# czbiohub-sf/yogo

Hardware: AMD Instinct MI355X
Metric: training images/sec (772x1032 gray) (higher is better)
Workload: dtype bf16; 1 GPU; BASELINE configs[2]: full train step (fwd+loss+bwd+clamp+AdamW), base_model, 772x1032x1 uint8, 7 classes; per_gpu_batch=128, global_batch=128, parallelism=dp1

## Files before the change

yogo_amd/csrc/conv_bf16_direct.hip:

```cpp
#include "common.h"
#ifndef YOGO_ST_AUX
#define YOGO_ST_AUX 2
#endif
#include <mutex>

#ifndef DD_ABL
#define DD_ABL 0
#endif
typedef unsigned int u32x4 __attribute__((ext_vector_type(4)));
typedef float f32x16 __attribute__((ext_vector_type(16)));
typedef __bf16 bf16x8 __attribute__((ext_vector_type(8)));

struct ConvDirectS2dParams {
  const u32x4* in;
  const u32x4* wp;
  u32x4* out;
  const unsigned char* signs;
  const float* chan_scale;
  int B, Kb, M, Mb, Mpad, IH, IW, OH, OW;
  int npass;
  int tiles_per_img, ntiles;
  unsigned m_iw, m_tpi;
};

namespace {
__device__ __forceinline__ int dd_udivm1(int n, int d, unsigned m) { return d == 1 ? n : (int)__umulhi((unsigned)n, m); }
}

template <int NK, int NMB, bool SIGNS>
__global__ __launch_bounds__(256 * NMB) __attribute__((amdgpu_waves_per_eu(NMB == 1 ? 4 : 2, NMB == 1 ? 4 : 2))) void conv_bf16_s2d_direct_kernel(
    const ConvDirectS2dParams p) {
  extern __shared__ __attribute__((aligned(16))) u32x4 lds_w[];
  constexpr int OOB = (int)0x80000000u;
  constexpr int KB = 2 * NK, MP = 32 * NMB, NT = 256 * NMB, NWV = 4 * NMB;
  const int tid = threadIdx.x, lane = tid & 63, l31 = lane & 31, half = lane >> 5;
  const int wave = __builtin_amdgcn_readfirstlane(tid >> 6);
  const int bid = blockIdx.x;
  const int xcd = bid & 7;
  const int pass = (bid >> 3) % p.npass;
  const int slot = bid / (8 * p.npass);
  const int nslot = gridDim.x / (8 * p.npass);
  const int t8 = (p.ntiles + 7) >> 3;
  const int t_end = min(p.ntiles, (xcd + 1) * t8);
  for (int i = tid; i < 9 * KB * MP; i += NT) {
    const int m = i % MP, r = i / MP;
    lds_w[i] = p.wp[(size_t)r * p.Mpad + pass * MP + m];
  }
  float* my_scale = reinterpret_cast<float*>(lds_w + 9 * KB * MP) + wave * MP;
  __syncthreads();
  const int IH = p.IH, IW = p.IW, OH = p.OH, OW = p.OW;
  const int kcb = IH * IW * 16, plane = OH * OW, plane16 = plane * 16, nq = IH * IW;
  const int sq = p.Mpad >> 4;
  const int ch0 = pass * MP;
  struct Geo {
    int b, pix;
    int vsh[4];
    bool qv, vx, vy;
  };
  auto geo_of = [&](int tile) __attribute__((always_inline)) {
    Geo g;
    g.b = dd_udivm1(tile, p.tiles_per_img, p.m_tpi);
    const int t = tile - g.b * p.tiles_per_img;
    const int q = t * 32 + l31;
    g.qv = q < nq;
    const int qc = g.qv ? q : nq - 1;
    const int a = dd_udivm1(qc, IW, p.m_iw), c = qc - a * IW;
    const bool cx = c + 1 < IW, cy = a + 1 < IH;
    g.vx = 2 * c + 1 < OW; g.vy = 2 * a + 1 < OH;
    const int v00 = (a * IW + c) * 16 + half * kcb;
    g.vsh[0] = v00; g.vsh[1] = cx ? v00 + 16 : OOB; g.vsh[2] = cy ? v00 + IW * 16 : OOB; g.vsh[3] = (cx && cy) ? v00 + IW * 16 + 16 : OOB;
    g.pix = 2 * a * OW + 2 * c;
    return g;
  };
  u32x4 Bq[2][4];
  auto load_step = [&](const Geo& g, int kc, u32x4 (&dst)[4]) __attribute__((always_inline)) {
    const auto rs_in = __builtin_amdgcn_make_buffer_rsrc((void*)(p.in + (size_t)g.b * KB * IH * IW), (short)0, KB * kcb, 0x00020000);
#pragma unroll
    for (int s = 0; s < 4; ++s) dst[s] = __builtin_bit_cast(u32x4, __builtin_amdgcn_raw_buffer_load_b128(rs_in, (DD_ABL & 4) ? OOB : g.vsh[s], (2 * kc) * kcb, 0));
  };
  static_assert(NK % 2 == 0, "the first operand set of the NEXT tile is requested while the last step still reads the second");
  const int tstep = nslot * NWV;
  int tile = xcd * t8 + slot * NWV + wave;
  Geo G = geo_of(min(tile, p.ntiles - 1));
  if (tile < t_end) load_step(G, 0, Bq[0]);
  for (; tile < t_end; tile += tstep) {
    const int b = G.b, pix = G.pix;
    const bool qv = G.qv, vx = G.vx, vy = G.vy;
    const auto rs_o = __builtin_amdgcn_make_buffer_rsrc((void*)(p.out + (size_t)b * p.Mb * plane), (short)0, p.Mb * plane16, 0x00020000);
    float my_s = 0.f;
    if (lane < MP) my_s = ch0 + lane < p.M ? (p.chan_scale != nullptr ? p.chan_scale[(size_t)b * p.M + ch0 + lane] : 1.f) : 0.f;
    unsigned sg[2][2] = {{0u, 0u}, {0u, 0u}};
    if constexpr (SIGNS) {
      const auto rs_s = __builtin_amdgcn_make_buffer_rsrc((void*)(p.signs + (size_t)b * plane * 2 * sq), (short)0, plane * 2 * sq, 0x00020000);
#pragma unroll
      for (int py = 0; py < 2; ++py)
#pragma unroll
        for (int px = 0; px < 2; ++px) {
          const bool ok = qv && (px == 0 || vx) && (py == 0 || vy);
          const int vs = ok ? (half * plane + pix + py * OW + px) * sq + pass * 2 * NMB : OOB;
          if constexpr (NMB == 2) sg[py][px] = (unsigned)__builtin_amdgcn_raw_buffer_load_b32(rs_s, vs, 0, 0);
          else sg[py][px] = (unsigned)__builtin_amdgcn_raw_buffer_load_b16(rs_s, vs, 0, 0);
        }
    }
    f32x16 acc[NMB][2][2];
#pragma unroll
    for (int mb = 0; mb < NMB; ++mb)
#pragma unroll
      for (int py = 0; py < 2; ++py)
#pragma unroll
        for (int px = 0; px < 2; ++px)
#pragma unroll
          for (int r = 0; r < 16; ++r) acc[mb][py][px][r] = 0.f;
#pragma unroll
    for (int kc = 0; kc < NK; ++kc) {
      if (kc + 1 < NK) load_step(G, kc + 1, Bq[(kc + 1) & 1]);
      const u32x4(&Bc)[4] = Bq[kc & 1];
      const u32x4* wk = lds_w + (2 * kc + half) * MP + l31;
#define DD_MF(PY, PX, S, SH)                                                                                                                     \
  _Pragma("unroll") for (int mb = 0; mb < NMB; ++mb) if (!(DD_ABL & 2)) acc[mb][PY][PX] = __builtin_amdgcn_mfma_f32_32x32x16_bf16(               \
      __builtin_bit_cast(bf16x8, (DD_ABL & 8) ? Bc[(SH) ^ 1] : wk[(S) * KB * MP + 32 * mb]), __builtin_bit_cast(bf16x8, Bc[SH]), acc[mb][PY][PX], 0, 0, 0); \
  else acc[mb][PY][PX][0] += __builtin_bit_cast(float, Bc[SH].x);
      __builtin_amdgcn_sched_barrier(0);
      DD_MF(0, 0, 0, 0) DD_MF(0, 1, 1, 0) DD_MF(1, 0, 3, 0)
      __builtin_amdgcn_sched_barrier(0);
      DD_MF(1, 1, 5, 0) DD_MF(0, 1, 2, 1) DD_MF(1, 1, 6, 1)
      __builtin_amdgcn_sched_barrier(0);
      DD_MF(1, 0, 4, 2) DD_MF(1, 1, 7, 2) DD_MF(1, 1, 8, 3)
      __builtin_amdgcn_sched_barrier(0);
#undef DD_MF
    }
    __builtin_amdgcn_sched_barrier(0);
    if (tile + tstep < t_end) {
      G = geo_of(tile + tstep);
      load_step(G, 0, Bq[0]);
    }
    __builtin_amdgcn_sched_barrier(0);
    if (lane < MP) my_scale[lane] = my_s;
#pragma unroll
    for (int mb = 0; mb < NMB; ++mb)
#pragma unroll
    for (int gp = 0; gp < 2; ++gp) {
      const int cb = pass * 4 * NMB + 4 * mb + 2 * gp;
      const int cl = 32 * mb + 16 * gp + 4 * half;
      const float4 sA = *reinterpret_cast<const float4*>(my_scale + cl), sB = *reinterpret_cast<const float4*>(my_scale + cl + 8);
      const float sa[8] = {sA.x, sA.y, sA.z, sA.w, sB.x, sB.y, sB.z, sB.w};
      float sl[8];
#pragma unroll
      for (int i = 0; i < 8; ++i) sl[i] = LEAKY_SLOPE * sa[i];
#pragma unroll
      for (int py = 0; py < 2; ++py) {
        u32x4 un[2];
#pragma unroll
        for (int px = 0; px < 2; ++px) {
          float v[8];
          if constexpr (SIGNS) {
            const unsigned m = sg[py][px] >> (8 * (2 * mb + gp));
#pragma unroll
            for (int i = 0; i < 8; ++i) {
              const int tt = (int)(m << (31 - i)) >> 31;
              unsigned f;
              asm("v_bfi_b32 %0, %1, %2, %3" : "=v"(f) : "v"(tt), "v"(sa[i]), "v"(sl[i]));
              v[i] = acc[mb][py][px][8 * gp + i] * __builtin_bit_cast(float, f);
            }
          } else {
#pragma unroll
            for (int i = 0; i < 8; ++i) v[i] = fmaf(acc[mb][py][px][8 * gp + i], sa[i], 0.f * sa[i]);
          }
          bf16x8 o;
#pragma unroll
          for (int i = 0; i < 8; ++i) o[i] = (__bf16)v[i];
          const u32x4 w = __builtin_bit_cast(u32x4, o);
          const auto r0 = __builtin_amdgcn_permlane32_swap(w.x, w.z, false, false);
          const auto r1 = __builtin_amdgcn_permlane32_swap(w.y, w.w, false, false);
          un[px] = u32x4{r0[0], r1[0], r0[1], r1[1]};
        }
        u32x4 se[2];
        {
          const auto x0 = __builtin_amdgcn_permlane32_swap(un[0].x, un[1].x, false, false);
          const auto x1 = __builtin_amdgcn_permlane32_swap(un[0].y, un[1].y, false, false);
          const auto x2 = __builtin_amdgcn_permlane32_swap(un[0].z, un[1].z, false, false);
          const auto x3 = __builtin_amdgcn_permlane32_swap(un[0].w, un[1].w, false, false);
          se[0] = u32x4{x0[0], x1[0], x2[0], x3[0]};
          se[1] = u32x4{x0[1], x1[1], x2[1], x3[1]};
        }
        const bool okp = qv && (half == 0 || vx) && (py == 0 || vy);
#pragma unroll
        for (int e = 0; e < 2; ++e)
          __builtin_amdgcn_raw_buffer_store_b128(se[e], rs_o, (okp && cb + e < p.Mb && !(DD_ABL & 1)) ? (pix + py * OW + half) * 16 + (cb + e) * plane16 : OOB, 0, YOGO_ST_AUX);
      }
    }
  }
}

bool conv_bf16_s2d_direct_eligible(int K, int M, int OH, int OW, int B) {
  if (M < 1 || !((M <= 32 && (K == 32 || K == 64)) || (M > 64 && M <= 128 && K == 128))) return false;
  if (OH < 2 || OW < 2 || B <= 0) return false;
  const long long IH = (OH + 1) / 2, IW = (OW + 1) / 2, Mb = ((M + 15) / 16) * 2;
  if ((long long)(K / 8) * IH * IW * 16 >= (1ll << 31) || Mb * OH * OW * 16 >= (1ll << 31) || (long long)B * ((IH * IW + 31) / 32) >= (1ll << 31)) return false;
  const long long tpi = (IH * IW + 31) / 32;
  if (!magic_div_exact(B * tpi - 1, (int)tpi) || !magic_div_exact(tpi * 32, (int)IW)) return false;
  return true;
}

int launch_conv_bf16_s2d_direct(const void* in, const void* packed, void* out, const void* signs, const float* chan_scale, int B, int K, int M, int IH, int IW,
                                int OH, int OW, hipStream_t stream) {
  static std::mutex mu;
  static int n_cu_of[64] = {0};
  static bool attr_set[64] = {false};
  int dev = 0;
  if (hipGetDevice(&dev) != hipSuccess || dev < 0 || dev >= 64) {
    yogo_set_error("conv_bf16_s2d_direct: hipGetDevice failed");
    return YOGO_ERR_HIP;
  }
  const int nmb = M <= 32 ? 1 : 2;
  const int lds = 9 * (K / 8) * 32 * nmb * 16 + 4 * nmb * 32 * nmb * 4;
  int n_cu;
  {
    std::lock_guard<std::mutex> lk(mu);
    if (n_cu_of[dev] == 0) {
      hipDeviceProp_t prop;
      n_cu_of[dev] = (hipGetDeviceProperties(&prop, dev) == hipSuccess && prop.multiProcessorCount > 0) ? prop.multiProcessorCount : 256;
    }
    n_cu = n_cu_of[dev];
    if (nmb == 2 && !attr_set[dev]) {
      hipError_t e = hipFuncSetAttribute(reinterpret_cast<const void*>(&conv_bf16_s2d_direct_kernel<8, 2, true>), hipFuncAttributeMaxDynamicSharedMemorySize, lds);
      if (e == hipSuccess) e = hipFuncSetAttribute(reinterpret_cast<const void*>(&conv_bf16_s2d_direct_kernel<8, 2, false>), hipFuncAttributeMaxDynamicSharedMemorySize, lds);
      if (e != hipSuccess) {
        yogo_set_error("conv_bf16_s2d_direct: hipFuncSetAttribute: %s", hipGetErrorString(e));
        return YOGO_ERR_HIP;
      }
      attr_set[dev] = true;
    }
  }
  ConvDirectS2dParams p{};
  p.in = reinterpret_cast<const u32x4*>(in); p.wp = reinterpret_cast<const u32x4*>(packed); p.out = reinterpret_cast<u32x4*>(out);
  p.signs = reinterpret_cast<const unsigned char*>(signs); p.chan_scale = chan_scale;
  p.B = B; p.Kb = K / 8; p.M = M; p.Mb = ((M + 15) / 16) * 2; p.Mpad = nmb == 1 ? 32 : 128; p.IH = IH; p.IW = IW; p.OH = OH; p.OW = OW;
  p.npass = p.Mpad / (32 * nmb);
  p.tiles_per_img = cdiv(IH * IW, 32);
  p.ntiles = B * p.tiles_per_img;
  auto magic = [](int d) -> unsigned { return d <= 1 ? 0xFFFFFFFFu : (unsigned)(((1ull << 32) + (unsigned)d - 1ull) / (unsigned)d); };
  p.m_iw = magic(IW); p.m_tpi = magic(p.tiles_per_img);
  if (p.ntiles <= 0) return YOGO_OK;
  const int t8 = cdiv(p.ntiles, 8);
  const int grid = nmb == 1 ? 8 * max(1, min(cdiv(t8, 4), 4 * n_cu / 8)) : 16 * max(1, min(cdiv(t8, 8), n_cu / 16));
  const bool sg = signs != nullptr;
#define DD_LAUNCH(NK, NMB, S) hipLaunchKernelGGL((conv_bf16_s2d_direct_kernel<NK, NMB, S>), dim3(grid), dim3(256 * NMB), lds, stream, p)
  if (K == 128) { if (sg) DD_LAUNCH(8, 2, true); else DD_LAUNCH(8, 2, false); }
  else if (K == 64) { if (sg) DD_LAUNCH(4, 1, true); else DD_LAUNCH(4, 1, false); }
  else { if (sg) DD_LAUNCH(2, 1, true); else DD_LAUNCH(2, 1, false); }
#undef DD_LAUNCH
  if (yogo_launch_log_enabled())
    yogo_launch_log("conv_bf16_s2d_direct_kernel<%d, %d, %s> | K=%d M=%d dy=%dx%d dx=%dx%d tiles=%d grid=%d lds=%d signs=%d scale=%d", K / 16, nmb, sg ? "true" : "false",
                    K, M, IH, IW, OH, OW, p.ntiles, grid, lds, sg, chan_scale != nullptr);
  YOGO_CHECK_LAUNCH("conv_bf16_s2d_direct");
  return YOGO_OK;
}
```

yogo_amd/csrc/conv_first_fused_bwd.hip:

```cpp
#include "common.h"
#include <mutex>
#include <type_traits>
#include <utility>

typedef unsigned int u32x4 __attribute__((ext_vector_type(4)));
typedef int i32x4 __attribute__((ext_vector_type(4)));
typedef float f32x4 __attribute__((ext_vector_type(4)));
typedef float f32x2 __attribute__((ext_vector_type(2)));
typedef __bf16 bf16x8 __attribute__((ext_vector_type(8)));

struct DgFirstParams {
  const u32x4* g;
  const u32x4* wp;
  const unsigned char* img;
  const unsigned short* signs;
  float* part;
  const u32x4* x;
  float* slab;
  float* bias_part;
  int B, H, W, Mpad, act, ncol;
  int tiles_per_row, tile_rows, seg, segs_per_img, nsegs;
  unsigned m_tpr, m_spi;
};

namespace {
constexpr int DF_NJ = 9, DF_PER = 2 * DF_NJ + 2, DF_COUT = 16;
__device__ __forceinline__ int df_udivm1(int n, int d, unsigned m) { return d == 1 ? n : (int)__umulhi((unsigned)n, m); }
__device__ __forceinline__ unsigned df_u(unsigned v) { return (unsigned)__builtin_amdgcn_readfirstlane((int)v); }
__device__ __forceinline__ i32x4 df_rsrc(const void* ptr, unsigned bytes) {
  const unsigned long long a = reinterpret_cast<unsigned long long>(ptr);
  return i32x4{(int)df_u((unsigned)a), (int)df_u((unsigned)(a >> 32) & 0xFFFFu), (int)df_u(bytes), 0x00020000};
}
__device__ __forceinline__ void df_dma16(i32x4 rs, unsigned lds_addr, int voff) {
  unsigned keep;
  lds_addr = df_u(lds_addr);
  asm volatile("s_mov_b32 %0, m0\n\ts_mov_b32 m0, %2\n\ts_nop 4\n\tbuffer_load_dwordx4 %1, %3, 0 offen lds\n\ts_mov_b32 m0, %0"
               : "=&s"(keep) : "v"(voff), "s"(lds_addr), "s"(rs) : "memory");
}
__device__ __forceinline__ void df_dma4(i32x4 rs, unsigned lds_addr, int voff) {
  unsigned keep;
  lds_addr = df_u(lds_addr);
  asm volatile("s_mov_b32 %0, m0\n\ts_mov_b32 m0, %2\n\ts_nop 4\n\tbuffer_load_dword %1, %3, 0 offen lds\n\ts_mov_b32 m0, %0"
               : "=&s"(keep) : "v"(voff), "s"(lds_addr), "s"(rs) : "memory");
}
__device__ __forceinline__ void df_wait_dma() { asm volatile("s_waitcnt vmcnt(0)" ::: "memory"); }
__device__ __forceinline__ bf16x8 df_tr8(const unsigned char* a, int second) {
  typedef __bf16 bf16x4 __attribute__((ext_vector_type(4)));
  typedef bf16x4 __attribute__((address_space(3))) * lds_v4;
  const bf16x4 lo = __builtin_amdgcn_ds_read_tr16_b64_v4bf16((lds_v4)(a));
  const bf16x4 hi = __builtin_amdgcn_ds_read_tr16_b64_v4bf16((lds_v4)(a + second));
  return __builtin_shufflevector(lo, hi, 0, 1, 2, 3, 4, 5, 6, 7);
}
}

#ifndef DF_WAVES_PER_EU
#define DF_WAVES_PER_EU 2
#endif
#ifndef DF_NPF
#define DF_NPF 6
#endif
#ifndef DF_NPF_WG
#define DF_NPF_WG 3
#endif
namespace {
template <class F, int... I>
__device__ __forceinline__ void df_static_for(F&& f, std::integer_sequence<int, I...>) {
  (f(std::integral_constant<int, I>{}), ...);
}
}
template <int R, int NWV, bool WG>
__global__ __launch_bounds__(64 * NWV) __attribute__((amdgpu_waves_per_eu(DF_WAVES_PER_EU))) void conv_bf16_dgrad_first_bwd_kernel(const DgFirstParams p) {
  extern __shared__ __attribute__((aligned(16))) u32x4 lds_u[];
  constexpr int OOB = (int)0x80000000u;
  constexpr int KB = 4, NR = R + 2, ROWU = 34, TU = KB * NR * ROWU, NDMA = (TU + 63) / 64;
  constexpr int IR = 2 * R + 1, IROWB = 72, IDW = IROWB / 4, IU = IR * IDW, NIDMA = (IU + 63) / 64;
  constexpr int SU = R * 16, NSDMA = (SU + 63) / 64;
  static_assert(!WG || (R % 2) == 0, "a piece of the staged x tile is two whole rows");
  constexpr int NXDMA = WG ? R : 0;
  constexpr int WAVE_BYTES = NDMA * 1024 + NIDMA * 256 + NSDMA * 256 + NXDMA * 1024;
  constexpr int CONST_BYTES = ((IR * IROWB + 15) / 16) * 16;
  const int tid = threadIdx.x, lane = tid & 63, c16 = lane & 15, g4 = lane >> 4;
  const int wave = __builtin_amdgcn_readfirstlane(tid >> 6);
  const int H = p.H, W = p.W, IH0 = 2 * H, IW0 = 2 * W;
  const int kcb = H * W * 16;
  const bool leaky = p.act == ACT_LEAKY;
  const unsigned my_addr = (unsigned)(wave * WAVE_BYTES), my_img_addr = my_addr + NDMA * 1024, my_sg_addr = my_img_addr + NIDMA * 256;
  [[maybe_unused]] const unsigned my_x_addr = my_sg_addr + NSDMA * 256;
  const unsigned ones_addr = (unsigned)(NWV * WAVE_BYTES), zeros_addr = ones_addr + CONST_BYTES;
  const u32x4* my_tile = lds_u + wave * (WAVE_BYTES / 16);
  const unsigned char* lds8 = reinterpret_cast<const unsigned char*>(lds_u);
  {
    unsigned* cw = reinterpret_cast<unsigned*>(lds_u) + ones_addr / 4;
    for (int e = tid; e < CONST_BYTES / 4; e += 64 * NWV) {
      cw[e] = 0x01010101u;
      cw[e + CONST_BYTES / 4] = 0u;
    }
  }
  __syncthreads();

  bf16x8 wv[9];
#pragma unroll
  for (int tp = 0; tp < 9; ++tp) wv[tp] = __builtin_bit_cast(bf16x8, p.wp[(tp * KB + g4) * p.Mpad + c16]);

  int rel[NDMA];
  unsigned rc[NDMA];
#pragma unroll
  for (int i = 0; i < NDMA; ++i) {
    const int u = i * 64 + lane;
    const int kb = u / (NR * ROWU), rem = u - kb * (NR * ROWU);
    const int r = rem / ROWU, cc = rem - r * ROWU;
    rel[i] = u < TU ? kb * kcb + (r * W + cc) * 16 : OOB;
    rc[i] = u < TU ? (unsigned)(r << 16 | cc) : 0xFFFFFFFFu;
  }
  unsigned irc[NIDMA];
#pragma unroll
  for (int i = 0; i < NIDMA; ++i) {
    const int e = i * 64 + lane;
    const int r = e / IDW, d = e - r * IDW;
    irc[i] = e < IU ? (unsigned)(r << 16 | d) : 0xFFFFFFFFu;
  }
  const int xj = c16 < 9 ? c16 : 0, kh = xj / 3, kw = xj - 3 * kh;
  const unsigned x_addr = c16 < 9 ? my_img_addr + (unsigned)(kh * IROWB + ((3 + 8 * g4 + kw) & ~3)) : (c16 == 9 ? ones_addr : zeros_addr) + (unsigned)(8 * g4);
  const unsigned x_sh = c16 < 9 ? (unsigned)((3 + kw) & 3) : 0u;
  const unsigned sg_addr = my_sg_addr + (unsigned)(8 * g4);
  const unsigned sg_pos = (unsigned)(c16 < 4 ? c16 : c16 < 8 ? c16 + 4 : c16 < 12 ? c16 - 4 : c16);

  f32x4 d2p = {0.f, 0.f, 0.f, 0.f}, d2n = {0.f, 0.f, 0.f, 0.f};
  f32x4 wacc[WG ? 2 : 1][WG ? 9 : 1], bacc[WG ? 2 : 1];
#pragma unroll
  for (int c = 0; c < (WG ? 2 : 1); ++c) {
    bacc[c] = f32x4{0.f, 0.f, 0.f, 0.f};
#pragma unroll
    for (int t = 0; t < (WG ? 9 : 1); ++t) wacc[c][t] = f32x4{0.f, 0.f, 0.f, 0.f};
  }
  [[maybe_unused]] const unsigned tr_g = my_addr + (unsigned)((((c16 & 3) >> 1) * NR * ROWU + 8 * g4 + (c16 >> 2)) * 16 + (c16 & 1) * 8);
  [[maybe_unused]] const unsigned tr_x = my_x_addr + (unsigned)((((c16 & 3) >> 1) * R * 32 + 8 * g4 + (c16 >> 2)) * 16 + (c16 & 1) * 8);
  const u32x4 ones_op = {0x3F803F80u, 0x3F803F80u, 0x3F803F80u, 0x3F803F80u};

  const int xcd = blockIdx.x & 7, slot = blockIdx.x >> 3, nslot = gridDim.x >> 3;
  const int s8 = (p.nsegs + 7) >> 3, s_end = min(p.nsegs, (xcd + 1) * s8);
  for (int sgm = xcd * s8 + slot * NWV + wave; sgm < s_end; sgm += nslot * NWV) {
    const int b = df_udivm1(sgm, p.segs_per_img, p.m_spi);
    const int t = sgm - b * p.segs_per_img;
    const int sy = df_udivm1(t, p.tiles_per_row, p.m_tpr), ox0 = (t - sy * p.tiles_per_row) * 32;
    const int ty_end = min(p.tile_rows, (sy + 1) * p.seg);
   for (int ty = sy * p.seg; ty < ty_end; ++ty) {
    const int oy0 = ty * R;
    {
      const i32x4 rs_g = df_rsrc(p.g + (size_t)b * KB * H * W, (unsigned)(KB * kcb));
      const int iy0 = oy0 - 1, ix0 = ox0 - 1;
      const int base = (iy0 * W + ix0) * 16;
      if (iy0 >= 0 && iy0 + NR <= H && ix0 >= 0 && ix0 + ROWU <= W) {
#pragma unroll
        for (int i = 0; i < NDMA; ++i) df_dma16(rs_g, my_addr + (unsigned)i * 1024u, (i + 1) * 64 <= TU ? rel[i] + base : (rel[i] == OOB ? OOB : rel[i] + base));
      } else {
#pragma unroll
        for (int i = 0; i < NDMA; ++i) {
          const int r = (int)(rc[i] >> 16), c = (int)(rc[i] & 0xFFFFu);
          const bool ok = ((unsigned)(iy0 + r) < (unsigned)H) && ((unsigned)(ix0 + c) < (unsigned)W);
          df_dma16(rs_g, my_addr + (unsigned)i * 1024u, ok ? rel[i] + base : OOB);
        }
      }
      const i32x4 rs_i = df_rsrc(p.img + (size_t)b * IH0 * IW0, (unsigned)(IH0 * IW0));
      const int jy0 = 2 * oy0 - 1, jx0 = 2 * ox0 - 4;
#pragma unroll
      for (int i = 0; i < NIDMA; ++i) {
        const int r = (int)(irc[i] >> 16), d = (int)(irc[i] & 0xFFFFu);
        const int iy = jy0 + r, ix = jx0 + 4 * d;
        const bool ok = ((unsigned)iy < (unsigned)IH0) && ((unsigned)ix < (unsigned)IW0);
        df_dma4(rs_i, my_img_addr + (unsigned)i * 256u, ok ? iy * IW0 + ix : OOB);
      }
      if (leaky) {
        const i32x4 rs_s = df_rsrc(p.signs + (size_t)b * H * W, (unsigned)(H * W * 2));
#pragma unroll
        for (int i = 0; i < NSDMA; ++i) {
          const int e = i * 64 + lane, r = e >> 4, d = e & 15;
          const bool ok = e < SU && oy0 + r < H && ox0 + 2 * d < W;
          df_dma4(rs_s, my_sg_addr + (unsigned)i * 256u, ok ? ((oy0 + r) * W + ox0 + 2 * d) * 2 : OOB);
        }
      }
      if constexpr (WG) {
        const i32x4 rs_x = df_rsrc(p.x + (size_t)b * 2 * H * W, (unsigned)(2 * kcb));
        const int hi = lane >> 5, col = lane & 31;
        const int xo = ((oy0 + hi) * W + ox0 + col) * 16;
        const bool cok = ox0 + col < W;
#pragma unroll
        for (int i = 0; i < NXDMA; ++i) {
          constexpr int dummy = 0; (void)dummy;
          const int kb = (2 * i) / R, row0 = (2 * i) % R;
          df_dma16(rs_x, my_x_addr + (unsigned)i * 1024u, (cok && oy0 + row0 + hi < H) ? xo + kb * kcb + row0 * W * 16 : OOB);
        }
      }
    }
    const bool right = ox0 + 32 > W;
    df_wait_dma();
    const u32x4* bt = my_tile + g4 * NR * ROWU + c16;
#pragma unroll
    for (int rr = 0; rr < R; ++rr) {
      if (oy0 + rr >= H) break;
      constexpr int NST = WG ? 36 : 18, NPF = WG ? DF_NPF_WG : DF_NPF;
      f32x4 acc[2];
      bf16x8 ring[NPF];
      [[maybe_unused]] bf16x8 xt;
      auto load = [&](auto s_tag) {
        constexpr int S = decltype(s_tag)::value;
        if constexpr (S < 18) {
          constexpr int pb = S / 9, tp = S % 9, ky = tp / 3, kx = tp % 3;
          ring[S % NPF] = __builtin_bit_cast(bf16x8, bt[(rr + ky) * ROWU + 16 * pb + kx]);
        } else {
          constexpr int cbk = (S - 18) / 9, tp = (S - 18) % 9, ky = tp / 3, kx = tp % 3;
          ring[S % NPF] = df_tr8(lds8 + tr_g + ((cbk * 2 * NR + rr + 2 - ky) * ROWU + 2 - kx) * 16, 64);
        }
      };
      auto use = [&](auto s_tag) {
        constexpr int S = decltype(s_tag)::value;
        if constexpr (S < 18) {
          constexpr int pb = S / 9, tp = S % 9;
          acc[pb] = __builtin_amdgcn_mfma_f32_16x16x32_bf16(ring[S % NPF], wv[tp], tp == 0 ? f32x4{0.f, 0.f, 0.f, 0.f} : acc[pb], 0, 0, 0);
        } else if constexpr (WG) {
          constexpr int cbk = (S - 18) / 9, tp = (S - 18) % 9;
          wacc[cbk][tp] = __builtin_amdgcn_mfma_f32_16x16x32_bf16(ring[S % NPF], xt, wacc[cbk][tp], 0, 0, 0);
          if constexpr (tp == 4) bacc[cbk] = __builtin_amdgcn_mfma_f32_16x16x32_bf16(ring[S % NPF], __builtin_bit_cast(bf16x8, ones_op), bacc[cbk], 0, 0, 0);
        }
      };
      unsigned xr[2][3];
      unsigned sw[2][2] = {{0xFFFFFFFFu, 0xFFFFFFFFu}, {0xFFFFFFFFu, 0xFFFFFFFFu}};
      u32x4 xop, gpos, gneg;
      auto p3 = [&](auto k_tag) {
        constexpr int K = decltype(k_tag)::value;
        typedef __bf16 bf16x2 __attribute__((ext_vector_type(2)));
        if constexpr (K == 0) {
#pragma unroll
          for (int pb = 0; pb < 2; ++pb) {
            const unsigned char* xa = lds8 + x_addr + rr * (2 * IROWB) + 32 * pb;
            xr[pb][0] = *reinterpret_cast<const unsigned*>(xa);
            xr[pb][1] = *reinterpret_cast<const unsigned*>(xa + 4);
            xr[pb][2] = *reinterpret_cast<const unsigned*>(xa + 8);
            if (leaky) {
              const unsigned long long s2 = *reinterpret_cast<const unsigned long long*>(lds8 + sg_addr + rr * 64 + 32 * pb);
              sw[pb][0] = (unsigned)s2;
              sw[pb][1] = (unsigned)(s2 >> 32);
            }
          }
        } else if constexpr (K == 1 || K == 2) {
          constexpr int pb = K - 1;
          const unsigned lo4 = __builtin_amdgcn_alignbyte(xr[pb][1], xr[pb][0], x_sh), hi4 = __builtin_amdgcn_alignbyte(xr[pb][2], xr[pb][1], x_sh);
          const unsigned xs = __builtin_amdgcn_perm(hi4, lo4, 0x06040200u);
          const bf16x2 q0 = {(__bf16)(float)(xs & 0xFFu), (__bf16)(float)((xs >> 8) & 0xFFu)};
          const bf16x2 q1 = {(__bf16)(float)((xs >> 16) & 0xFFu), (__bf16)(float)(xs >> 24)};
          xop[2 * pb] = __builtin_bit_cast(unsigned, q0);
          xop[2 * pb + 1] = __builtin_bit_cast(unsigned, q1);
        } else if constexpr (K == 3 || K == 4) {
          constexpr int pb = K - 3;
#pragma unroll
          for (int q = 0; q < 2; ++q) {
            const bf16x2 dq = {(__bf16)acc[pb][2 * q], (__bf16)acc[pb][2 * q + 1]};
            unsigned dw = __builtin_bit_cast(unsigned, dq);
            if (right && ox0 + 16 * pb + 4 * g4 + 2 * q >= W) dw = 0u;
            const unsigned m = leaky ? __umul24((sw[pb][q] >> sg_pos) & 0x00010001u, 0xFFFFu) : 0xFFFFFFFFu;
            const unsigned pos = dw & m;
            gpos[2 * pb + q] = pos;
            gneg[2 * pb + q] = dw ^ pos;
          }
        } else if constexpr (K == 5) {
          d2p = __builtin_amdgcn_mfma_f32_16x16x32_bf16(__builtin_bit_cast(bf16x8, xop), __builtin_bit_cast(bf16x8, gpos), d2p, 0, 0, 0);
        } else {
          d2n = __builtin_amdgcn_mfma_f32_16x16x32_bf16(__builtin_bit_cast(bf16x8, xop), __builtin_bit_cast(bf16x8, gneg), d2n, 0, 0, 0);
        }
      };
      df_static_for([&](auto s_tag) { load(s_tag); }, std::make_integer_sequence<int, NPF>{});
      __builtin_amdgcn_sched_barrier(0);
      df_static_for(
          [&](auto s_tag) {
            constexpr int S = decltype(s_tag)::value;
            use(s_tag);
            if constexpr (S + NPF < NST) load(std::integral_constant<int, S + NPF>{});
            if constexpr (WG) {
              if constexpr (S == 10) xt = df_tr8(lds8 + tr_x + rr * 512, 64);
              if constexpr (S == 18) p3(std::integral_constant<int, 0>{});
              if constexpr (S == 23) p3(std::integral_constant<int, 1>{});
              if constexpr (S == 25) p3(std::integral_constant<int, 2>{});
              if constexpr (S == 27) p3(std::integral_constant<int, 3>{});
              if constexpr (S == 29) p3(std::integral_constant<int, 4>{});
              if constexpr (S == 31) p3(std::integral_constant<int, 5>{});
              if constexpr (S == 32) p3(std::integral_constant<int, 6>{});
            } else {
              if constexpr (S == 12) p3(std::integral_constant<int, 0>{});
              if constexpr (S == 15) p3(std::integral_constant<int, 1>{});
              if constexpr (S == 16) p3(std::integral_constant<int, 2>{});
            }
            __builtin_amdgcn_sched_barrier(0);
          },
          std::make_integer_sequence<int, NST>{});
      if constexpr (!WG) {
        p3(std::integral_constant<int, 3>{});
        p3(std::integral_constant<int, 4>{});
        p3(std::integral_constant<int, 5>{});
        p3(std::integral_constant<int, 6>{});
      }
    }
   }
  }
  float* prow = p.part + (size_t)(blockIdx.x * NWV + wave) * p.ncol;
#pragma unroll
  for (int i = 0; i < 4; ++i) {
    const int j = 4 * g4 + i;
    const float v = d2p[i] + LEAKY_SLOPE * d2n[i];
    if (j < DF_NJ) prow[c16 * DF_PER + j] = v;
    else if (j == DF_NJ) prow[c16 * DF_PER + 2 * DF_NJ] = v;
  }
  if (g4 == 0) prow[c16 * DF_PER + 2 * DF_NJ + 1] = 0.f;
  for (int e = lane; e < DF_COUT * DF_NJ; e += 64) prow[(e / DF_NJ) * DF_PER + DF_NJ + e % DF_NJ] = 0.f;
  for (int e = lane; e < DF_NJ + DF_NJ * DF_NJ; e += 64) prow[DF_COUT * DF_PER + e] = 0.f;
  if constexpr (WG) {
    constexpr int NE = 9 * 32 * 16, STRIDE = NE + 32;
    static_assert(NWV * STRIDE * 4 <= NWV * WAVE_BYTES + 2 * CONST_BYTES, "the reduction uses the kernel's LDS allocation");
    __syncthreads();
    float* red = reinterpret_cast<float*>(lds_u) + wave * STRIDE;
#pragma unroll
    for (int cbk = 0; cbk < 2; ++cbk)
#pragma unroll
      for (int i = 0; i < 4; ++i) {
        const int co = 16 * cbk + 4 * g4 + i;
#pragma unroll
        for (int tp = 0; tp < 9; ++tp) red[(tp * 32 + co) * 16 + c16] = wacc[cbk][tp][i];
        if (c16 == 0) red[NE + co] = bacc[cbk][i];
      }
    __syncthreads();
    const float* r0 = reinterpret_cast<const float*>(lds_u);
    float* sl = p.slab + (size_t)blockIdx.x * NE;
    float* bp = p.bias_part + (size_t)blockIdx.x * 32;
    for (int e = tid; e < STRIDE; e += 64 * NWV) {
      float v = r0[e];
#pragma unroll
      for (int w = 1; w < NWV; ++w) v += r0[w * STRIDE + e];
      if (e < NE) sl[e] = v;
      else bp[e - NE] = v;
    }
  }
}

#ifndef DF_TILE_ROWS
#define DF_TILE_ROWS 6
#endif
#ifndef DF_TILE_ROWS_WG
#define DF_TILE_ROWS_WG 4
#endif
#ifndef DF_WAVES
#define DF_WAVES 4
#endif
namespace {
constexpr int DF_NWV = DF_WAVES;
constexpr int df_rows(bool wg) { return wg ? DF_TILE_ROWS_WG : DF_TILE_ROWS; }
constexpr int df_lds_bytes(int R, int NWV, bool wg) {
  return NWV * (((4 * (R + 2) * 34 + 63) / 64) * 1024 + (((2 * R + 1) * 18 + 63) / 64) * 256 + ((R * 16 + 63) / 64) * 256 + (wg ? R * 1024 : 0)) +
         2 * ((((2 * R + 1) * 72 + 15) / 16) * 16);
}
int df_n_cu() {
  static std::mutex mu;
  static int n_cu_of[64] = {0};
  int dev = 0;
  if (hipGetDevice(&dev) != hipSuccess || dev < 0 || dev >= 64) return -1;
  std::lock_guard<std::mutex> lk(mu);
  if (n_cu_of[dev] == 0) {
    hipDeviceProp_t prop;
    n_cu_of[dev] = (hipGetDeviceProperties(&prop, dev) == hipSuccess && prop.multiProcessorCount > 0) ? prop.multiProcessorCount : 256;
  }
  return n_cu_of[dev];
}
struct DfPlan { int grid, seg; };
DfPlan df_plan(int B, int H, int W, int n_cu, bool wg) {
  const int R = df_rows(wg);
  const int nty = cdiv(H, R), ntx = cdiv(W, 32);
  const int lds = df_lds_bytes(R, DF_NWV, wg);
  const int per_cu = max(1, min(16 / DF_NWV, (160 * 1024) / lds));
#ifdef DF_SEG
  const int seg_lo = DF_SEG, seg_hi = DF_SEG;
#else
  const int seg_lo = 1, seg_hi = 16;
#endif
  DfPlan best{8, 1};
  double best_cost = -1.0;
  for (int seg = seg_lo; seg <= seg_hi && (seg <= nty || seg == seg_lo); ++seg) {
    const long long nsegs = (long long)B * cdiv(nty, seg) * ntx;
    const int s8 = (int)((nsegs + 7) / 8);
    const int grid = 8 * max(1, min(cdiv(s8, DF_NWV), per_cu * n_cu / 8));
    const int waves_per_xcd = grid / 8 * DF_NWV;
    const double cost = (double)cdiv(s8, waves_per_xcd) * min(seg, nty) * (1.0 + (2.0 / R) / min(seg, nty));
    if (best_cost < 0 || cost < best_cost) { best_cost = cost; best = DfPlan{grid, seg}; }
  }
  return best;
}
bool df_shape_ok(int Cmid, int Cout1, int H, int W, int B, int act0, bool wg) {
  if (Cmid != 16 || Cout1 != 32 || H < 1 || W < 2 || (W & 1) || B < 1 || (act0 != ACT_NONE && act0 != ACT_LEAKY)) return false;
  const int R = df_rows(wg);
  if ((long long)4 * H * W * 16 >= (1ll << 31) || (long long)4 * H * W >= (1ll << 31) || (long long)B * cdiv(H, R) * cdiv(W, 32) >= (1ll << 31)) return false;
  const long long tpr = cdiv(W, 32);
  for (int seg = 1; seg <= 16; ++seg) {
    const long long spi = (long long)cdiv(cdiv(H, R), seg) * tpr;
    if (!magic_div_exact((long long)B * spi - 1, (int)spi) || !magic_div_exact(spi, (int)tpr)) return false;
  }
  return true;
}

template <bool WG>
int df_launch(DgFirstParams p, int B, int H, int W, int act0, const char* what, hipStream_t stream) {
  const int n_cu = df_n_cu();
  if (n_cu < 0) {
    yogo_set_error("%s: hipGetDevice failed", what);
    return YOGO_ERR_HIP;
  }
  constexpr int R = df_rows(WG);
  p.B = B; p.H = H; p.W = W; p.Mpad = 32; p.act = act0; p.ncol = DF_COUT * DF_PER + DF_NJ + DF_NJ * DF_NJ;
  const DfPlan pl = df_plan(B, H, W, n_cu, WG);
  p.tiles_per_row = cdiv(W, 32); p.tile_rows = cdiv(H, R); p.seg = pl.seg;
  p.segs_per_img = cdiv(p.tile_rows, pl.seg) * p.tiles_per_row; p.nsegs = B * p.segs_per_img;
  auto magic = [](int d) -> unsigned { return d <= 1 ? 0xFFFFFFFFu : (unsigned)(((1ull << 32) + (unsigned)d - 1ull) / (unsigned)d); };
  p.m_tpr = magic(p.tiles_per_row); p.m_spi = magic(p.segs_per_img);
  const int grid = pl.grid;
  constexpr int lds = df_lds_bytes(R, DF_NWV, WG);
  static_assert(lds <= 160 * 1024, "LDS");
  if (lds > 64 * 1024) {
    static std::mutex mu;
    static bool done[64] = {};
    int dev = 0;
    (void)hipGetDevice(&dev);
    std::lock_guard<std::mutex> lk(mu);
    if (dev >= 0 && dev < 64 && !done[dev]) {
      hipError_t e = hipFuncSetAttribute(reinterpret_cast<const void*>(&conv_bf16_dgrad_first_bwd_kernel<R, DF_NWV, WG>), hipFuncAttributeMaxDynamicSharedMemorySize, lds);
      if (e != hipSuccess) {
        yogo_set_error("%s: hipFuncSetAttribute: %s", what, hipGetErrorString(e));
        return YOGO_ERR_HIP;
      }
      done[dev] = true;
    }
  }
  hipLaunchKernelGGL((conv_bf16_dgrad_first_bwd_kernel<R, DF_NWV, WG>), dim3(grid), dim3(64 * DF_NWV), lds, stream, p);
  if (yogo_launch_log_enabled())
    yogo_launch_log("conv_bf16_dgrad_first_bwd_kernel<%d, %d, %s> | K=32 M=16 at %dx%d segments=%d of %d tiles grid=%d lds=%d act0=%d", R, DF_NWV, WG ? "true" : "false", H, W,
                    p.nsegs, pl.seg, grid, lds, act0);
  hipError_t e = hipGetLastError();
  if (e != hipSuccess) {
    yogo_set_error("%s: launch failed: %s", what, hipGetErrorString(e));
    return YOGO_ERR_HIP;
  }
  return YOGO_OK;
}
}

extern "C" int yogo_internal_wgrad_reduce_q(void* queue, const float* slab, int nslab, int T, int M, int N, int Mpad, int Npad, float clip, float* dw,
                                            const float* bias_part, int nbias, float* db, hipStream_t stream);

extern "C" int yogo_conv2d_dgrad_first_bwd_supported(int Cmid, int Cout1, int H, int W, int B, int act0) {
  return (df_shape_ok(Cmid, Cout1, H, W, B, act0, false) && df_shape_ok(Cmid, Cout1, H, W, B, act0, true)) ? 1 : 0;
}

extern "C" int yogo_conv2d_dgrad_first_bwd_rows(int B, int H, int W, int with_wgrad, int* rows) {
  YOGO_CHECK_ARG(rows && B > 0 && H > 0 && W > 0, "conv2d_dgrad_first_bwd_rows: bad arguments");
  const int n_cu = df_n_cu();
  if (n_cu < 0) {
    yogo_set_error("conv2d_dgrad_first_bwd_rows: hipGetDevice failed");
    return YOGO_ERR_HIP;
  }
  *rows = df_plan(B, H, W, n_cu, with_wgrad != 0).grid * DF_NWV;
  return YOGO_OK;
}

extern "C" int yogo_conv2d_dgrad_bf16_first_bwd(const void* g, const void* packed, const void* image, const void* signs, float* part, int B, int Cmid,
                                                int Cout1, int H, int W, int act0, hipStream_t stream) {
  YOGO_CHECK_ARG(g && packed && image && part, "conv2d_dgrad_bf16_first_bwd: null pointer");
  YOGO_CHECK_ARG(yogo_conv2d_dgrad_first_bwd_supported(Cmid, Cout1, H, W, B, act0), "conv2d_dgrad_bf16_first_bwd: unsupported shape");
  YOGO_CHECK_ARG(signs != nullptr || act0 == ACT_NONE, "conv2d_dgrad_bf16_first_bwd: LeakyReLU needs the sign map");
  DgFirstParams p{};
  p.g = reinterpret_cast<const u32x4*>(g); p.wp = reinterpret_cast<const u32x4*>(packed); p.img = reinterpret_cast<const unsigned char*>(image);
  p.signs = reinterpret_cast<const unsigned short*>(signs); p.part = part;
  return df_launch<false>(p, B, H, W, act0, "conv2d_dgrad_bf16_first_bwd", stream);
}

extern "C" int yogo_conv2d_dgrad_wgrad_first_bwd_workspace_bytes(int B, int H, int W, size_t* bytes) {
  YOGO_CHECK_ARG(bytes && B > 0 && H > 0 && W > 0, "conv2d_dgrad_wgrad_first_bwd_workspace_bytes: bad arguments");
  const int n_cu = df_n_cu();
  if (n_cu < 0) {
    yogo_set_error("conv2d_dgrad_wgrad_first_bwd_workspace_bytes: hipGetDevice failed");
    return YOGO_ERR_HIP;
  }
  *bytes = (size_t)df_plan(B, H, W, n_cu, true).grid * (9 * 32 * 16 + 32) * sizeof(float);
  return YOGO_OK;
}
extern "C" int yogo_conv2d_dgrad_wgrad_bf16_first_bwd(const void* g, const void* packed, const void* x, const void* image, const void* signs, float* part,
                                                      float* dw, float* db, void* workspace, int B, int Cmid, int Cout1, int H, int W, int act0, float clip,
                                                      void* queue, hipStream_t stream) {
  YOGO_CHECK_ARG(g && packed && x && image && part && dw && workspace, "conv2d_dgrad_wgrad_bf16_first_bwd: null pointer");
  YOGO_CHECK_ARG(yogo_conv2d_dgrad_first_bwd_supported(Cmid, Cout1, H, W, B, act0), "conv2d_dgrad_wgrad_bf16_first_bwd: unsupported shape");
  YOGO_CHECK_ARG(signs != nullptr || act0 == ACT_NONE, "conv2d_dgrad_wgrad_bf16_first_bwd: LeakyReLU needs the sign map");
  const int n_cu = df_n_cu();
  if (n_cu < 0) {
    yogo_set_error("conv2d_dgrad_wgrad_bf16_first_bwd: hipGetDevice failed");
    return YOGO_ERR_HIP;
  }
  const int rows = df_plan(B, H, W, n_cu, true).grid;
  DgFirstParams p{};
  p.g = reinterpret_cast<const u32x4*>(g); p.wp = reinterpret_cast<const u32x4*>(packed); p.img = reinterpret_cast<const unsigned char*>(image);
  p.signs = reinterpret_cast<const unsigned short*>(signs); p.part = part;
  p.x = reinterpret_cast<const u32x4*>(x); p.slab = reinterpret_cast<float*>(workspace); p.bias_part = p.slab + (size_t)rows * 9 * 32 * 16;
  if (int e = df_launch<true>(p, B, H, W, act0, "conv2d_dgrad_wgrad_bf16_first_bwd", stream)) return e;
  return yogo_internal_wgrad_reduce_q(queue, p.slab, rows, 9, Cout1, Cmid, 32, 16, clip, dw, p.bias_part, rows, db, stream);
}
```

Baseline: 11230 images/s.

## Add configurable load ring depth and trickled stores to direct s2d conv kernel

Generalizes the double-buffered input operand prefetch into a configurable ring of depth D, with an unrolled tile loop when D does not divide NK. Adds an optional mode that defers output stores into the next tile's K loop, plus an optional wave stagger. The channel-scale load becomes a buffer load. The defaults keep ring depth 2 with trickling and stagger off, but change NMB==1 occupancy from 4 to 3 waves per EU and shrink the grid to match. That trades fewer resident waves for more registers per wave.

```diff
diff --git a/yogo_amd/csrc/conv_bf16_direct.hip b/yogo_amd/csrc/conv_bf16_direct.hip
--- a/yogo_amd/csrc/conv_bf16_direct.hip
+++ b/yogo_amd/csrc/conv_bf16_direct.hip
@@ -3,9 +3,25 @@
 #define YOGO_ST_AUX 2
 #endif
 #include <mutex>
+#include <type_traits>
 
 #ifndef DD_ABL
 #define DD_ABL 0
+#endif
+#ifndef DD_RING2
+#define DD_RING2 2
+#endif
+#ifndef DD_RING1
+#define DD_RING1 2
+#endif
+#ifndef DD_TRICKLE
+#define DD_TRICKLE 0
+#endif
+#ifndef DD_WPE1
+#define DD_WPE1 3
+#endif
+#ifndef DD_STAGGER
+#define DD_STAGGER 0
 #endif
 typedef unsigned int u32x4 __attribute__((ext_vector_type(4)));
 typedef float f32x16 __attribute__((ext_vector_type(16)));
@@ -28,7 +44,7 @@
 }
 
 template <int NK, int NMB, bool SIGNS>
-__global__ __launch_bounds__(256 * NMB) __attribute__((amdgpu_waves_per_eu(NMB == 1 ? 4 : 2, NMB == 1 ? 4 : 2))) void conv_bf16_s2d_direct_kernel(
+__global__ __launch_bounds__(256 * NMB) __attribute__((amdgpu_waves_per_eu(NMB == 1 ? DD_WPE1 : 2, NMB == 1 ? DD_WPE1 : 2))) void conv_bf16_s2d_direct_kernel(
     const ConvDirectS2dParams p) {
   extern __shared__ __attribute__((aligned(16))) u32x4 lds_w[];
   constexpr int OOB = (int)0x80000000u;
@@ -48,6 +64,9 @@
   }
   float* my_scale = reinterpret_cast<float*>(lds_w + 9 * KB * MP) + wave * MP;
   __syncthreads();
+#if DD_STAGGER
+  for (int i = (NMB == 2 ? (wave >> 2) * 2 : (slot & 3)) * DD_STAGGER; i > 0; --i) __builtin_amdgcn_s_sleep(127);
+#endif
   const int IH = p.IH, IW = p.IW, OH = p.OH, OW = p.OW;
   const int kcb = IH * IW * 16, plane = OH * OW, plane16 = plane * 16, nq = IH * IW;
   const int sq = p.Mpad >> 4;
@@ -72,23 +91,55 @@
     g.pix = 2 * a * OW + 2 * c;
     return g;
   };
-  u32x4 Bq[2][4];
+  constexpr int DREQ = NMB == 1 ? DD_RING1 : DD_RING2;
+  constexpr int D = DREQ < 2 ? 2 : (DREQ > NK ? NK : DREQ);
+  constexpr bool TRICKLE = ((DD_TRICKLE) >> (NMB - 1)) & 1;
+  constexpr int TFRONT = NMB == 2 ? 2 : 0;
+  constexpr int NST = 8 * NMB;
+  constexpr bool LATE = D == 2;
+  static_assert(NK % D == 0 || D == 3, "a tile moves the ring by NK slots: D divides NK, or the tile loop is unrolled over the three rotations");
+  static_assert(NST % NK == 0, "the trickled stores of a tile leave in equal shares per K step");
+  u32x4 Bq[D][4];
   auto load_step = [&](const Geo& g, int kc, u32x4 (&dst)[4]) __attribute__((always_inline)) {
     const auto rs_in = __builtin_amdgcn_make_buffer_rsrc((void*)(p.in + (size_t)g.b * KB * IH * IW), (short)0, KB * kcb, 0x00020000);
 #pragma unroll
     for (int s = 0; s < 4; ++s) dst[s] = __builtin_bit_cast(u32x4, __builtin_amdgcn_raw_buffer_load_b128(rs_in, (DD_ABL & 4) ? OOB : g.vsh[s], (2 * kc) * kcb, 0));
   };
-  static_assert(NK % 2 == 0, "the first operand set of the NEXT tile is requested while the last step still reads the second");
+  auto geo_next = [&](int tile) __attribute__((always_inline)) {
+    Geo g = geo_of(min(tile, p.ntiles - 1));
+    if (tile >= t_end) g.vsh[0] = g.vsh[1] = g.vsh[2] = g.vsh[3] = OOB;
+    return g;
+  };
+  u32x4 pu[TRICKLE ? NST : 1];
+#pragma unroll
+  for (int i = 0; i < (TRICKLE ? NST : 1); ++i) pu[i] = u32x4{0u, 0u, 0u, 0u};
+  int pvo[2] = {OOB, OOB};
+  auto prs = __builtin_amdgcn_make_buffer_rsrc((void*)p.out, (short)0, 0, 0x00020000);
+  auto store_pending = [&](int i0, int i1) __attribute__((always_inline)) {
+#pragma unroll
+    for (int i = i0; i < i1; ++i) {
+      const int e = i & 1, py = (i >> 1) & 1, gp = (i >> 2) & 1, mb = i >> 3;
+      const int cbe = pass * 4 * NMB + 4 * mb + 2 * gp + e;
+      __builtin_amdgcn_raw_buffer_store_b128(pu[TRICKLE ? i : 0], prs, (pvo[py] != OOB && cbe < p.Mb && !(DD_ABL & 1)) ? pvo[py] + cbe * plane16 : OOB, 0, YOGO_ST_AUX);
+    }
+  };
   const int tstep = nslot * NWV;
   int tile = xcd * t8 + slot * NWV + wave;
-  Geo G = geo_of(min(tile, p.ntiles - 1));
-  if (tile < t_end) load_step(G, 0, Bq[0]);
-  for (; tile < t_end; tile += tstep) {
+  Geo G = geo_next(tile);
+#pragma unroll
+  for (int j = 0; j < D - 1; ++j) load_step(G, j, Bq[j]);
+  auto do_tile = [&](auto off_c) __attribute__((always_inline)) {
+    constexpr int OFF = decltype(off_c)::value;
     const int b = G.b, pix = G.pix;
     const bool qv = G.qv, vx = G.vx, vy = G.vy;
     const auto rs_o = __builtin_amdgcn_make_buffer_rsrc((void*)(p.out + (size_t)b * p.Mb * plane), (short)0, p.Mb * plane16, 0x00020000);
     float my_s = 0.f;
-    if (lane < MP) my_s = ch0 + lane < p.M ? (p.chan_scale != nullptr ? p.chan_scale[(size_t)b * p.M + ch0 + lane] : 1.f) : 0.f;
+    if (p.chan_scale != nullptr) {
+      const auto rs_c = __builtin_amdgcn_make_buffer_rsrc((void*)(p.chan_scale + (size_t)b * p.M), (short)0, p.M * 4, 0x00020000);
+      my_s = __builtin_bit_cast(float, __builtin_amdgcn_raw_buffer_load_b32(rs_c, lane < MP ? (ch0 + lane) * 4 : OOB, 0, 0));
+    } else if (lane < MP) {
+      my_s = ch0 + lane < p.M ? 1.f : 0.f;
+    }
     unsigned sg[2][2] = {{0u, 0u}, {0u, 0u}};
     if constexpr (SIGNS) {
       const auto rs_s = __builtin_amdgcn_make_buffer_rsrc((void*)(p.signs + (size_t)b * plane * 2 * sq), (short)0, plane * 2 * sq, 0x00020000);
@@ -111,10 +162,14 @@
         for (int px = 0; px < 2; ++px)
 #pragma unroll
           for (int r = 0; r < 16; ++r) acc[mb][py][px][r] = 0.f;
+    Geo Gn = G;
 #pragma unroll
     for (int kc = 0; kc < NK; ++kc) {
-      if (kc + 1 < NK) load_step(G, kc + 1, Bq[(kc + 1) & 1]);
-      const u32x4(&Bc)[4] = Bq[kc & 1];
+      if (kc == NK - D + 1 && !LATE) Gn = geo_next(tile + tstep);
+      if (kc + D - 1 < NK) load_step(G, kc + D - 1, Bq[(OFF + kc + D - 1) % D]);
+      else if (!LATE) load_step(Gn, kc + D - 1 - NK, Bq[(OFF + kc + D - 1) % D]);
+      if constexpr (TRICKLE) store_pending(kc == 0 ? 0 : min(NST, kc * (NST / NK) + TFRONT), min(NST, (kc + 1) * (NST / NK) + TFRONT));
+      const u32x4(&Bc)[4] = Bq[(OFF + kc) % D];
       const u32x4* wk = lds_w + (2 * kc + half) * MP + l31;
 #define DD_MF(PY, PX, S, SH)                                                                                                                     \
   _Pragma("unroll") for (int mb = 0; mb < NMB; ++mb) if (!(DD_ABL & 2)) acc[mb][PY][PX] = __builtin_amdgcn_mfma_f32_32x32x16_bf16(               \
@@ -130,12 +185,21 @@
 #undef DD_MF
     }
     __builtin_amdgcn_sched_barrier(0);
-    if (tile + tstep < t_end) {
-      G = geo_of(tile + tstep);
-      load_step(G, 0, Bq[0]);
-    }
-    __builtin_amdgcn_sched_barrier(0);
+    if constexpr (LATE) {
+      if (tile + tstep < t_end) {
+        G = geo_of(tile + tstep);
+        load_step(G, 0, Bq[(OFF + NK) % D]);
+      }
+      __builtin_amdgcn_sched_barrier(0);
+    } else {
+      G = Gn;
+    }
     if (lane < MP) my_scale[lane] = my_s;
+    if constexpr (TRICKLE) {
+      prs = rs_o;
+#pragma unroll
+      for (int py = 0; py < 2; ++py) pvo[py] = (qv && (half == 0 || vx) && (py == 0 || vy)) ? (pix + py * OW + half) * 16 : OOB;
+    }
 #pragma unroll
     for (int mb = 0; mb < NMB; ++mb)
 #pragma unroll
@@ -185,11 +249,29 @@
         }
         const bool okp = qv && (half == 0 || vx) && (py == 0 || vy);
 #pragma unroll
-        for (int e = 0; e < 2; ++e)
-          __builtin_amdgcn_raw_buffer_store_b128(se[e], rs_o, (okp && cb + e < p.Mb && !(DD_ABL & 1)) ? (pix + py * OW + half) * 16 + (cb + e) * plane16 : OOB, 0, YOGO_ST_AUX);
+        for (int e = 0; e < 2; ++e) {
+          if constexpr (TRICKLE) pu[TRICKLE ? ((mb * 2 + gp) * 2 + py) * 2 + e : 0] = se[e];
+          else __builtin_amdgcn_raw_buffer_store_b128(se[e], rs_o, (okp && cb + e < p.Mb && !(DD_ABL & 1)) ? (pix + py * OW + half) * 16 + (cb + e) * plane16 : OOB, 0, YOGO_ST_AUX);
+        }
       }
     }
+  };
+  if constexpr (NK % D == 0) {
+    for (; tile < t_end; tile += tstep) do_tile(std::integral_constant<int, 0>{});
+  } else {
+    for (;;) {
+      if (tile >= t_end) break;
+      do_tile(std::integral_constant<int, 0>{});
+      tile += tstep;
+      if (tile >= t_end) break;
+      do_tile(std::integral_constant<int, NK % D>{});
+      tile += tstep;
+      if (tile >= t_end) break;
+      do_tile(std::integral_constant<int, (2 * NK) % D>{});
+      tile += tstep;
+    }
   }
+  if constexpr (TRICKLE) store_pending(0, NST);
 }
 
 bool conv_bf16_s2d_direct_eligible(int K, int M, int OH, int OW, int B) {
@@ -243,7 +325,7 @@
   p.m_iw = magic(IW); p.m_tpi = magic(p.tiles_per_img);
   if (p.ntiles <= 0) return YOGO_OK;
   const int t8 = cdiv(p.ntiles, 8);
-  const int grid = nmb == 1 ? 8 * max(1, min(cdiv(t8, 4), 4 * n_cu / 8)) : 16 * max(1, min(cdiv(t8, 8), n_cu / 16));
+  const int grid = nmb == 1 ? 8 * max(1, min(cdiv(t8, 4), DD_WPE1 * n_cu / 8)) : 16 * max(1, min(cdiv(t8, 8), n_cu / 16));
   const bool sg = signs != nullptr;
 #define DD_LAUNCH(NK, NMB, S) hipLaunchKernelGGL((conv_bf16_s2d_direct_kernel<NK, NMB, S>), dim3(grid), dim3(256 * NMB), lds, stream, p)
   if (K == 128) { if (sg) DD_LAUNCH(8, 2, true); else DD_LAUNCH(8, 2, false); }
```

New measurement: 11220 images/s. No clear change (-0.0%).

## Reuse halo rows of gradient tile across tile rows via LDS ring buffer

Applied to the files above, without the earlier changes.

Changes the LDS layout of the staged gradient tile from channel-block-major to row-major slots, with each row padded to 36 units, and treats the NR row slots as a ring. Within a segment, each later tile row now loads only the R new rows and keeps the two overlapping halo rows from the previous tile instead of reloading all R+2 rows. This cuts global-to-LDS DMA traffic per tile. In exchange it adds per-row slot address computation and a slightly larger LDS footprint from the padding, and it adds test hooks to force the segment length.

```diff
diff --git a/yogo_amd/csrc/conv_first_fused_bwd.hip b/yogo_amd/csrc/conv_first_fused_bwd.hip
--- a/yogo_amd/csrc/conv_first_fused_bwd.hip
+++ b/yogo_amd/csrc/conv_first_fused_bwd.hip
@@ -72,7 +72,7 @@
 __global__ __launch_bounds__(64 * NWV) __attribute__((amdgpu_waves_per_eu(DF_WAVES_PER_EU))) void conv_bf16_dgrad_first_bwd_kernel(const DgFirstParams p) {
   extern __shared__ __attribute__((aligned(16))) u32x4 lds_u[];
   constexpr int OOB = (int)0x80000000u;
-  constexpr int KB = 4, NR = R + 2, ROWU = 34, TU = KB * NR * ROWU, NDMA = (TU + 63) / 64;
+  constexpr int KB = 4, NR = R + 2, ROWU = 34, KBU = 36, SLOTU = KB * KBU, TU = NR * SLOTU, NDMA = (TU + 63) / 64;
   constexpr int IR = 2 * R + 1, IROWB = 72, IDW = IROWB / 4, IU = IR * IDW, NIDMA = (IU + 63) / 64;
   constexpr int SU = R * 16, NSDMA = (SU + 63) / 64;
   static_assert(!WG || (R % 2) == 0, "a piece of the staged x tile is two whole rows");
@@ -87,7 +87,6 @@
   const unsigned my_addr = (unsigned)(wave * WAVE_BYTES), my_img_addr = my_addr + NDMA * 1024, my_sg_addr = my_img_addr + NIDMA * 256;
   [[maybe_unused]] const unsigned my_x_addr = my_sg_addr + NSDMA * 256;
   const unsigned ones_addr = (unsigned)(NWV * WAVE_BYTES), zeros_addr = ones_addr + CONST_BYTES;
-  const u32x4* my_tile = lds_u + wave * (WAVE_BYTES / 16);
   const unsigned char* lds8 = reinterpret_cast<const unsigned char*>(lds_u);
   {
     unsigned* cw = reinterpret_cast<unsigned*>(lds_u) + ones_addr / 4;
@@ -107,10 +106,10 @@
 #pragma unroll
   for (int i = 0; i < NDMA; ++i) {
     const int u = i * 64 + lane;
-    const int kb = u / (NR * ROWU), rem = u - kb * (NR * ROWU);
-    const int r = rem / ROWU, cc = rem - r * ROWU;
-    rel[i] = u < TU ? kb * kcb + (r * W + cc) * 16 : OOB;
-    rc[i] = u < TU ? (unsigned)(r << 16 | cc) : 0xFFFFFFFFu;
+    const int r = u / SLOTU, rem = u - r * SLOTU;
+    const int kb = rem / KBU, cc = rem - kb * KBU;
+    rel[i] = cc < ROWU ? kb * kcb + (r * W + cc) * 16 : OOB;
+    rc[i] = (unsigned)(r << 16 | cc);
   }
   unsigned irc[NIDMA];
 #pragma unroll
@@ -133,7 +132,8 @@
 #pragma unroll
     for (int t = 0; t < (WG ? 9 : 1); ++t) wacc[c][t] = f32x4{0.f, 0.f, 0.f, 0.f};
   }
-  [[maybe_unused]] const unsigned tr_g = my_addr + (unsigned)((((c16 & 3) >> 1) * NR * ROWU + 8 * g4 + (c16 >> 2)) * 16 + (c16 & 1) * 8);
+  [[maybe_unused]] const unsigned tr_g = my_addr + (unsigned)((((c16 & 3) >> 1) * KBU + 8 * g4 + (c16 >> 2)) * 16 + (c16 & 1) * 8);
+  const unsigned bt_g = my_addr + (unsigned)((g4 * KBU + c16) * 16);
   [[maybe_unused]] const unsigned tr_x = my_x_addr + (unsigned)((((c16 & 3) >> 1) * R * 32 + 8 * g4 + (c16 >> 2)) * 16 + (c16 & 1) * 8);
   const u32x4 ones_op = {0x3F803F80u, 0x3F803F80u, 0x3F803F80u, 0x3F803F80u};
 
@@ -144,21 +144,43 @@
     const int t = sgm - b * p.segs_per_img;
     const int sy = df_udivm1(t, p.tiles_per_row, p.m_tpr), ox0 = (t - sy * p.tiles_per_row) * 32;
     const int ty_end = min(p.tile_rows, (sy + 1) * p.seg);
-   for (int ty = sy * p.seg; ty < ty_end; ++ty) {
+   const int ty0 = sy * p.seg;
+   int phase = 0;
+   for (int ty = ty0; ty < ty_end; ++ty) {
     const int oy0 = ty * R;
     {
       const i32x4 rs_g = df_rsrc(p.g + (size_t)b * KB * H * W, (unsigned)(KB * kcb));
-      const int iy0 = oy0 - 1, ix0 = ox0 - 1;
-      const int base = (iy0 * W + ix0) * 16;
-      if (iy0 >= 0 && iy0 + NR <= H && ix0 >= 0 && ix0 + ROWU <= W) {
-#pragma unroll
-        for (int i = 0; i < NDMA; ++i) df_dma16(rs_g, my_addr + (unsigned)i * 1024u, (i + 1) * 64 <= TU ? rel[i] + base : (rel[i] == OOB ? OOB : rel[i] + base));
-      } else {
-#pragma unroll
-        for (int i = 0; i < NDMA; ++i) {
-          const int r = (int)(rc[i] >> 16), c = (int)(rc[i] & 0xFFFFu);
-          const bool ok = ((unsigned)(iy0 + r) < (unsigned)H) && ((unsigned)(ix0 + c) < (unsigned)W);
-          df_dma16(rs_g, my_addr + (unsigned)i * 1024u, ok ? rel[i] + base : OOB);
+      int s0 = 0, r0 = 0, n0 = NR, n1 = 0;
+      if (ty != ty0) {
+        phase = phase + R >= NR ? phase + R - NR : phase + R;
+        s0 = phase + 2 >= NR ? phase + 2 - NR : phase + 2;
+        r0 = 2;
+        n0 = min(R, NR - s0);
+        n1 = R - n0;
+      }
+      const int ix0 = ox0 - 1;
+      const bool cols_in = ix0 >= 0 && ix0 + ROWU <= W;
+#pragma nounroll
+      for (int run = 0; run < 2; ++run) {
+        const int n = run ? n1 : n0;
+        if (n == 0) break;
+        const int iy0 = oy0 - 1 + (run ? r0 + n0 : r0), lim = n * SLOTU;
+        const unsigned dst = my_addr + (unsigned)((run ? 0 : s0) * SLOTU * 16);
+        const int base = (iy0 * W + ix0) * 16;
+        if (cols_in && iy0 >= 0 && iy0 + n <= H) {
+#pragma unroll
+          for (int i = 0; i < NDMA; ++i)
+            if (i * 64 < lim) {
+              if (i * 64 + lane < lim) df_dma16(rs_g, dst + (unsigned)i * 1024u, rel[i] + base);
+            }
+        } else {
+#pragma unroll
+          for (int i = 0; i < NDMA; ++i)
+            if (i * 64 < lim) {
+              const int r = (int)(rc[i] >> 16), c = (int)(rc[i] & 0xFFFFu);
+              const bool ok = rel[i] != OOB && ((unsigned)(iy0 + r) < (unsigned)H) && ((unsigned)(ix0 + c) < (unsigned)W);
+              if (i * 64 + lane < lim) df_dma16(rs_g, dst + (unsigned)i * 1024u, ok ? rel[i] + base : OOB);
+            }
         }
       }
       const i32x4 rs_i = df_rsrc(p.img + (size_t)b * IH0 * IW0, (unsigned)(IH0 * IW0));
@@ -194,7 +216,14 @@
     }
     const bool right = ox0 + 32 > W;
     df_wait_dma();
-    const u32x4* bt = my_tile + g4 * NR * ROWU + c16;
+    unsigned row_b[NR];
+    [[maybe_unused]] unsigned row_t[NR];
+#pragma unroll
+    for (int r = 0; r < NR; ++r) {
+      const unsigned so = (unsigned)((phase + r >= NR ? phase + r - NR : phase + r) * SLOTU * 16);
+      row_b[r] = bt_g + so;
+      row_t[r] = tr_g + so;
+    }
 #pragma unroll
     for (int rr = 0; rr < R; ++rr) {
       if (oy0 + rr >= H) break;
@@ -206,10 +235,10 @@
         constexpr int S = decltype(s_tag)::value;
         if constexpr (S < 18) {
           constexpr int pb = S / 9, tp = S % 9, ky = tp / 3, kx = tp % 3;
-          ring[S % NPF] = __builtin_bit_cast(bf16x8, bt[(rr + ky) * ROWU + 16 * pb + kx]);
+          ring[S % NPF] = __builtin_bit_cast(bf16x8, *reinterpret_cast<const u32x4*>(lds8 + row_b[rr + ky] + (16 * pb + kx) * 16));
         } else {
           constexpr int cbk = (S - 18) / 9, tp = (S - 18) % 9, ky = tp / 3, kx = tp % 3;
-          ring[S % NPF] = df_tr8(lds8 + tr_g + ((cbk * 2 * NR + rr + 2 - ky) * ROWU + 2 - kx) * 16, 64);
+          ring[S % NPF] = df_tr8(lds8 + row_t[rr + 2 - ky] + (cbk * 2 * KBU + 2 - kx) * 16, 64);
         }
       };
       auto use = [&](auto s_tag) {
@@ -353,7 +382,7 @@
 constexpr int DF_NWV = DF_WAVES;
 constexpr int df_rows(bool wg) { return wg ? DF_TILE_ROWS_WG : DF_TILE_ROWS; }
 constexpr int df_lds_bytes(int R, int NWV, bool wg) {
-  return NWV * (((4 * (R + 2) * 34 + 63) / 64) * 1024 + (((2 * R + 1) * 18 + 63) / 64) * 256 + ((R * 16 + 63) / 64) * 256 + (wg ? R * 1024 : 0)) +
+  return NWV * ((((R + 2) * 4 * 36 + 63) / 64) * 1024 + (((2 * R + 1) * 18 + 63) / 64) * 256 + ((R * 16 + 63) / 64) * 256 + (wg ? R * 1024 : 0)) +
          2 * ((((2 * R + 1) * 72 + 15) / 16) * 16);
 }
 int df_n_cu() {
@@ -369,12 +398,17 @@
   return n_cu_of[dev];
 }
 struct DfPlan { int grid, seg; };
+#ifdef YOGO_TEST_HOOKS
+int g_df_seg = 0;
+#endif
 DfPlan df_plan(int B, int H, int W, int n_cu, bool wg) {
   const int R = df_rows(wg);
   const int nty = cdiv(H, R), ntx = cdiv(W, 32);
   const int lds = df_lds_bytes(R, DF_NWV, wg);
   const int per_cu = max(1, min(16 / DF_NWV, (160 * 1024) / lds));
-#ifdef DF_SEG
+#if defined(YOGO_TEST_HOOKS)
+  const int seg_lo = g_df_seg ? g_df_seg : 1, seg_hi = g_df_seg ? g_df_seg : 16;
+#elif defined(DF_SEG)
   const int seg_lo = DF_SEG, seg_hi = DF_SEG;
 #else
   const int seg_lo = 1, seg_hi = 16;
@@ -420,6 +454,7 @@
   const int grid = pl.grid;
   constexpr int lds = df_lds_bytes(R, DF_NWV, WG);
   static_assert(lds <= 160 * 1024, "LDS");
+  static_assert(!(WG && R == 4 && DF_NWV == 4) || lds <= 80 * 1024, "the benched instantiation keeps two workgroups per CU");
   if (lds > 64 * 1024) {
     static std::mutex mu;
     static bool done[64] = {};
@@ -506,3 +541,11 @@
   if (int e = df_launch<true>(p, B, H, W, act0, "conv2d_dgrad_wgrad_bf16_first_bwd", stream)) return e;
   return yogo_internal_wgrad_reduce_q(queue, p.slab, rows, 9, Cout1, Cmid, 32, 16, clip, dw, p.bias_part, rows, db, stream);
 }
+
+#ifdef YOGO_TEST_HOOKS
+extern "C" int yogo_hook_first_bwd_seg(int seg) {
+  YOGO_CHECK_ARG(seg >= 0 && seg <= 16, "hook_first_bwd_seg: 0 (the plan) or 1 .. 16");
+  g_df_seg = seg;
+  return YOGO_OK;
+}
+#endif
```

Result: no change. 10860 images/s before, 10850 images/s after (-0.1%).
